# jinkakei/q-gcm

Hardware: AMD Instinct MI355X
Metric: ocean timesteps/sec (NAtl 5km 3-layer qgostep+ocinvq+ocqbdy) (higher is better)
Workload: dtype f64; 1 GPU; double_gyre_ocean_only NAtl 5km, 961x961x3 p-grid, dto=540s, Gaussian-eddy IC + double-gyre wind, oml off; parallelism=single GPU

## Files before the change

### q-gcm_amd/csrc/k_dst64.h

```cpp
#pragma once
#include "qgcm_dev.h"
#include "k_dst.h"
#include "k_misc.h"

#pragma clang fp contract(fast)

#ifndef D64_WAVES
#define D64_WAVES 2
#endif
#define D64_NT (64 * D64_WAVES)
#define D64_ROW 72

__device__ __forceinline__ void wave_lds_sync() {
  __builtin_amdgcn_fence(__ATOMIC_SEQ_CST, "wavefront");
  __builtin_amdgcn_wave_barrier();
}

__device__ __forceinline__ cplx cscale(cplx a, double s) { return {a.x * s, a.y * s}; }
__device__ __forceinline__ cplx cmpi(cplx a) { return {-a.y, a.x}; }

__device__ __forceinline__ void dft8(cplx *x) {
  const double r2 = 0.70710678118654752440;
  cplx e0 = cadd(x[0], x[4]), o0 = csub(x[0], x[4]);
  cplx e1 = cadd(x[1], x[5]), o1 = csub(x[1], x[5]);
// ... 73 lines not shown
  for (int ka = 0; ka < 3; ++ka)
#pragma unroll
    for (int kb = 0; kb < 5; ++kb) t[ka + 3 * kb] = a[5 * ka + kb];
#pragma unroll
  for (int k = 0; k < 15; ++k) a[k] = t[k];
}

template <int CTRL, int ROWMASK>
__device__ __forceinline__ double d64_dpp(double v) {
  int lo = __double2loint(v), hi = __double2hiint(v);
  lo = __builtin_amdgcn_update_dpp(0, lo, CTRL, ROWMASK, 0xf, true);
  hi = __builtin_amdgcn_update_dpp(0, hi, CTRL, ROWMASK, 0xf, true);
  return __hiloint2double(hi, lo);
}
__device__ __forceinline__ void d64_wave_scan2(double &a, double &b) {
  a += d64_dpp<0x111, 0xf>(a); b += d64_dpp<0x111, 0xf>(b);
  a += d64_dpp<0x112, 0xf>(a); b += d64_dpp<0x112, 0xf>(b);
  a += d64_dpp<0x114, 0xf>(a); b += d64_dpp<0x114, 0xf>(b);
  a += d64_dpp<0x118, 0xf>(a); b += d64_dpp<0x118, 0xf>(b);
  a += d64_dpp<0x142, 0xa>(a); b += d64_dpp<0x142, 0xa>(b);
  a += d64_dpp<0x143, 0xc>(a); b += d64_dpp<0x143, 0xc>(b);
}

template <int M>
__device__ __forceinline__ void dst64_front(const QgDstParams &P, const double *rowa, const double *rowb, bool has_b,
                                            cplx *F, cplx *W64, int lane) {
  constexpr int N = 64 * M, n = N - 1, NS2 = n / 2;

  cplx tw1[M];
  {
    double2 w = P.twid[lane];
    tw1[1 % M] = {w.x, w.y};
#pragma unroll
    for (int k1 = 2; k1 < M; ++k1) tw1[k1] = cmul(tw1[k1 / 2], tw1[k1 - k1 / 2]);
  }
  {
    double2 w = P.twid[M * lane];
    W64[lane] = {w.x, w.y};
  }

  constexpr int MH = M / 2;
  cplx a[M];
  {
    const double *rb = has_b ? rowb : rowa;
    const double bsc = has_b ? 1.0 : 0.0;
    double snv[MH + 1], xav[MH + 1], xac[MH + 1], xbv[MH + 1], xbc[MH + 1];
#pragma unroll
    for (int n1 = 0; n1 <= MH; ++n1) {
      const int j = 64 * n1 + lane;
      const int k = (j <= NS2 + 1) ? j : 0;
      const int i1 = k > 0 ? k - 1 : 0, i2 = k > 0 ? n - k : 0;
      snv[n1] = P.sintab[(k <= NS2) ? k : 0];
      xav[n1] = rowa[i1];
      xac[n1] = rowa[i2];
      xbv[n1] = rb[i1];
      xbc[n1] = rb[i2];
    }
    const int ml = (64 - lane) & 63;
#pragma unroll
    for (int n1 = 0; n1 <= MH; ++n1) {
      const int j = 64 * n1 + lane;
      const double va = xav[n1], ca = xac[n1], vb = bsc * xbv[n1], cb = bsc * xbc[n1];
      const double sn = snv[n1];
      const double t1a = va - ca, t2a = sn * (va + ca);
      const double t1b = vb - cb, t2b = sn * (vb + cb);
      cplx z = {t1a + t2a, t1b + t2b};
      if (j == NS2 + 1) z = {4.0 * va, 4.0 * vb};
      if (j == 0) z = {0.0, 0.0};
      a[n1] = z;
      if (j >= 1 && j <= NS2) {
        const int mn1 = (lane == 0) ? M - n1 : M - 1 - n1;
        F[mn1 * D64_ROW + ml + (ml >> 3)] = {t2a - t1a, t2b - t1b};
      }
    }
    wave_lds_sync();
#pragma unroll
    for (int n1 = MH; n1 < M; ++n1) {
      const int j = 64 * n1 + lane;
      const cplx zz = F[n1 * D64_ROW + lane + (lane >> 3)];
      if (j >= NS2 + 2) a[n1] = zz;
    }
    wave_lds_sync();
  }
  dftM<M>(a);
#pragma unroll
// ... 180 lines not shown
      const int t = lane + 64 * u;
      if (t < N / 2) {
        qg_store16_wt(rowa + 2 * t, oa[u].x, oa[u].y);
        if (has_b) qg_store16_wt(rowb + 2 * t, ob[u].x, ob[u].y);
      }
    }
  }
  QG_STAMP(0, 3);
  QG_STAMP_DRAIN();
  QG_STAMP(0, 4);
  if (ROWSUM) {
#pragma unroll
    for (int off = 32; off > 0; off >>= 1) {
      rsa += __shfl_down(rsa, off);
      rsb += __shfl_down(rsb, off);
    }
    if (lane == 0) {
      P.rowsum[(long)m * ny + (ja - 1)] = rsa;
      if (has_b) P.rowsum[(long)m * ny + ja] = rsb;
    }
  }
}

#pragma clang fp contract(off)

template <int M, int NL, bool BDY, bool HALO, bool CONSTR, bool AVG = false>
__global__ __launch_bounds__(64 * (NL + (CONSTR ? 1 : 0))) void k_dst64_unpack(const QgDstParams P, const QgUnpackParams U,
                                                                                      const QgBdyParams B, const QgConstrLite C) {
  constexpr int N = 64 * M, NP = N + N / 16;
  __shared__ __align__(16) cplx Fsh[NL][M * D64_ROW];
  __shared__ __align__(16) cplx W64sh[NL][64];
  __shared__ double hc_sh[NL];
  const int tid = threadIdx.x;
  const int lane = tid & 63;
  const int wv = __builtin_amdgcn_readfirstlane(tid >> 6);
  const int ldw = P.g.ldw;
  const int ja = P.g.jr0 + 2 * blockIdx.x;
  const bool has_b = (ja + 1 <= P.g.jr1);
  const long fs = U.g.fstride;
  const int nx = U.g.nx, nyg = U.g.nyg, joff = U.g.joff;
  constexpr int NX = N + 1;
  double hc[NL];
  const int jlo = U.g.jlo, jhi = U.g.jhi, ldxm = U.g.ldx;
  auto msg_p = [&](int gi, int gj, const double *pl) {
    if (HALO && U.msg_lo && gj - jlo < 3) {
#pragma unroll
      for (int k = 0; k < NL; ++k) U.msg_lo[((long)k * 3 + (gj - jlo)) * ldxm + (gi - 1)] = pl[k];
    }
    if (HALO && U.msg_hi && jhi - gj < 3) {
#pragma unroll
      for (int k = 0; k < NL; ++k) U.msg_hi[((long)k * 3 + (gj - (jhi - 2))) * ldxm + (gi - 1)] = pl[k];
    }
// ... 90 lines not shown
    constr_xin<NL>(C, lane, xin);
#pragma unroll
    for (int k = 0; k < NL - 1; ++k) dpn[k] = C.sc->dpioc[k];
    constr_box_solve<NL>(C, xin, dpn, x);
    if (lane == 0) {
#pragma unroll
      for (int m = 1; m < NL; ++m) hc_sh[m] = x[m - 1];
      if (blockIdx.x == 0) {
#pragma unroll
        for (int m = 0; m < NL; ++m) C.sc->xinhom[m] = xin[m];
#pragma unroll
        for (int k = 0; k < NL - 1; ++k) C.sc->hclco[k] = x[k];
      }
    }
    __syncthreads();
#pragma unroll
    for (int m = 1; m < NL; ++m) hc[m] = x[m - 1];
    if (lane < 2) wall_columns(lane, w);
    return;
  }
  constexpr int NT = 64 * NL, NPAIR = (NX - 3) / 2, NIT = (NPAIR + NT - 1) / NT;
  const double *rowa = P.wrk + P.g.wstride * wv + (long)(ja - 1) * ldw;
  QG_STAMP(2, 0);
  dst64_front<M>(P, rowa, rowa + ldw, has_b, Fsh[wv], W64sh[wv], lane);
  QG_STAMP(2, 1);
  asm volatile("" ::: "memory");
  double2 oc[2][NIT][NL - 1];
#pragma unroll
  for (int r = 0; r < 2; ++r)
#pragma unroll
    for (int it = 0; it < NIT; ++it) {
      const int q = tid + it * NT;
      const int gi = 3 + 2 * q;
      const bool ok = q < NPAIR && (r == 0 || has_b);
      const long o = (long)(ja + r - 1) * U.g.ldx + (gi - 1);
#pragma unroll
      for (int m = 1; m < NL; ++m) oc[r][it][m - 1] = ok ? *reinterpret_cast<const double2 *>(U.ochom + fs * (m - 1) + o) : double2{0.0, 0.0};
    }
  double2 pcv[AVG ? 2 : 1][AVG ? NIT : 1][AVG ? NL : 1];
  if (AVG) {
#pragma unroll
    for (int r = 0; r < 2; ++r)
#pragma unroll
      for (int it = 0; it < NIT; ++it) {
        const int q = tid + it * NT, qc = q < NPAIR ? q : 0;
        const long o = (long)(ja + ((r == 0 || has_b) ? r : 0) - 1) * U.g.ldx + (3 + 2 * qc - 1);
#pragma unroll
// ... 104 lines not shown
```

### q-gcm_amd/csrc/k_misc.h

```cpp
#pragma once
#include "qgcm_dev.h"

#define CS_NT 256

__device__ inline void qg_lu_solve(int n, const double *lu, const int *piv, double *b) {
  for (int k = 0; k < n; ++k)
    if (piv[k] != k) {
      double t = b[k];
      b[k] = b[piv[k]];
      b[piv[k]] = t;
    }
  for (int k = 0; k < n; ++k)
    for (int i = k + 1; i < n; ++i) b[i] -= lu[i + n * k] * b[k];
  for (int k = n - 1; k >= 0; --k) {
    b[k] /= lu[k + n * k];
    for (int i = 0; i < k; ++i) b[i] -= lu[i + n * k] * b[k];
  }
}

__device__ inline double qg_block_sum(double v, double *red, int tid) {
  red[tid] = v;
  __syncthreads();
  for (int off = CS_NT / 2; off > 0; off >>= 1) {
    if (tid < off) red[tid] += red[tid + off];
// ... 40 lines not shown
    double aitmp = sc->dpioc[k];
    sc->dpioc[k] = sc->dpiocp[k] - tdto * gpoc[k] * aient;
    sc->dpiocp[k] = aitmp;
  }
}

template <int NL, class PT>
__device__ __forceinline__ void constr_box_solve(const PT &P, const double *xin, const double *dpn, double *x) {
  constexpr int n1 = NL - 1;
  double rhs[n1], r[n1], w[n1];
#pragma unroll
  for (int k = 0; k < n1; ++k) {
    double rhsum = 0.0;
#pragma unroll
    for (int m = 0; m < NL; ++m) rhsum = rhsum + P.cs.cdiffo[m + NL * k] * xin[m];
    rhs[k] = dpn[k] - rhsum;
    x[k] = rhs[k];
  }
  auto lu_solve = [&](double *b) {
#pragma unroll
    for (int k = 0; k < n1; ++k) {
      const int pk = P.cs.ipiv[k];
#pragma unroll
      for (int i = 0; i < n1; ++i)
        if (i > k && i == pk) {
          double t = b[k];
          b[k] = b[i];
          b[i] = t;
        }
    }
#pragma unroll
    for (int k = 0; k < n1; ++k)
#pragma unroll
      for (int i = k + 1; i < n1; ++i) b[i] -= P.cs.cdhlu[i + n1 * k] * b[k];
#pragma unroll
    for (int k = n1 - 1; k >= 0; --k) {
      b[k] /= P.cs.cdhlu[k + n1 * k];
#pragma unroll
      for (int i = 0; i < k; ++i) b[i] -= P.cs.cdhlu[i + n1 * k] * b[k];
    }
  };
  lu_solve(x);
  const double eps = 1.1102230246251565e-16, safmin = 2.2250738585072014e-308;
  const double safe1 = (n1 + 1) * safmin, safe2 = safe1 / eps;
  double lstres = 3.0;
  for (int count = 1;; ++count) {
#pragma unroll
    for (int i = 0; i < n1; ++i) {
      double sv = rhs[i], t = fabs(rhs[i]);
#pragma unroll
      for (int j = 0; j < n1; ++j) {
        sv -= P.cs.cdhoc[i + n1 * j] * x[j];
// ... 261 lines not shown
```

### q-gcm_amd/csrc/k_thomas.h

```cpp
#pragma once
#include "qgcm_dev.h"
#include "k_cyclic.h"

#define TH_KW 16
#define TH_NC 64
#define TH_NT (TH_KW * TH_NC)
static_assert(TH_NC == 64, "the chunk scan maps the 64 chunks of a wavenumber to the lanes of one wave");

template <int CTRL>
__device__ __forceinline__ double th_dpp(double v) {
  int lo = __double2loint(v), hi = __double2hiint(v);
  lo = __builtin_amdgcn_update_dpp(lo, lo, CTRL, 0xf, 0xf, false);
  hi = __builtin_amdgcn_update_dpp(hi, hi, CTRL, 0xf, 0xf, false);
  return __hiloint2double(hi, lo);
}
template <int CTRL>
__device__ __forceinline__ void th_scan_step(double &Cs, double &Ds, bool take) {
  const double Cp = th_dpp<CTRL>(Cs), Dp = th_dpp<CTRL>(Ds);
  if (take) {
    Cs = Cs + Ds * Cp;
    Ds = Ds * Dp;
  }
}
__device__ __forceinline__ void affine_scan(double &Cs, double &Ds, int lane) {
  const int rl = lane & 15;
  th_scan_step<0x111>(Cs, Ds, rl >= 1);
  th_scan_step<0x112>(Cs, Ds, rl >= 2);
  th_scan_step<0x114>(Cs, Ds, rl >= 4);
  th_scan_step<0x118>(Cs, Ds, rl >= 8);
  th_scan_step<0x142>(Cs, Ds, (lane & 16) != 0);
  th_scan_step<0x143>(Cs, Ds, lane >= 32);
}

#define TH_MSG 3
#define TH_CST 4
template <int R, int PHASE, bool CYCA = false, int KW = TH_KW>
__global__ __launch_bounds__(KW * TH_NC, (KW == 8 && R <= 16) ? 4 : 1) void k_thomas(const QgThomasParams P) {
  static_assert(TH_KW % KW == 0, "a workgroup's wavenumbers lie inside one block of the pivot tables");
  static_assert(KW % 2 == 0, "the write-through stores pair the lanes of neighbouring wavenumbers");
  __shared__ double sC[TH_NC][KW + 1];
  __shared__ double sD[TH_NC][KW + 1];
  __shared__ double sIn[TH_NC][KW + 1];
  const int tid = threadIdx.x;
  if (CYCA && blockIdx.x == gridDim.x - 1) {
    if (P.cycq && blockIdx.y == 0 && tid < 64) {
      double a4[QG_MAXL], b4[QG_MAXL];
      switch (P.g.nl) {
        case 2: constr_cyc_partA<2>(*P.cycq, tid, a4, b4); break;
        case 3: constr_cyc_partA<3>(*P.cycq, tid, a4, b4); break;
        default: constr_cyc_partA<4>(*P.cycq, tid, a4, b4); break;
      }
    }
    return;
  }
  QG_STAMP(1, 0);
  int bxl = (int)blockIdx.x;
  if (KW == 8) {
    const int nfull = ((int)gridDim.x - (CYCA ? 1 : 0)) / 16 * 16;
    if (bxl < nfull) bxl = (bxl & ~15) + 2 * (bxl & 7) + ((bxl >> 3) & 1);
  }
  const int kk = tid % KW;
  const int c = tid / KW;
  const int lane = tid & 63, wv = tid >> 6;
  const int k = bxl * KW + kk;
  const int kq = bxl * KW + wv;
  const int m = blockIdx.y + P.layer0;
  const int nr = P.g.jr1 - P.g.jr0 + 1;
  const int ldw = P.g.ldw;
  const bool kok = k < P.g.nk;
  const double a = P.aoc;
  const int r0 = c * R;
  const long mk = TH_MSG * ((long)m * ldw + kq);
  const double ft = P.ftnorm;

  const double *wbase_c = P.wrk + P.g.wstride * m + (long)(P.g.jr0 - 1) * ldw + bxl * KW;
  double *wbase = const_cast<double *>(wbase_c);
  const unsigned off0 = (unsigned)(r0 * ldw + kk);
  constexpr bool PRED = (PHASE != 0);
  double w[R], b[R];
#pragma unroll
  for (int t = 0; t < R; ++t) {
    int r = r0 + t;
    const bool ok = kok && r < nr && PHASE != 4 && PHASE != 5;
    w[t] = ok ? wbase[off0 + (unsigned)(t * ldw)] : 0.0;
  }
  {
    const int tb = m * P.nblk + (bxl * KW) / TH_KW;
    const int rcb = P.rcb[tb];
    const double binf = kok ? P.binf[(long)m * ldw + k] : 0.0;
#pragma unroll
    for (int t = 0; t < R; ++t) b[t] = binf;
    if (r0 < rcb) {
      const double *tab = P.ptab + (long)P.poff[tb] * TH_KW + (bxl * KW) % TH_KW + kk;
#pragma unroll
      for (int t = 0; t < R; ++t) {
        const int r = r0 + t;
        const int rc = r < rcb ? r : rcb - 1;
        const double v = tab[rc * TH_KW];
        b[t] = (r < rcb && kok) ? v : binf;
      }
    }
    if (r0 + R > nr) {
#pragma unroll
      for (int t = 0; t < R; ++t)
        if (r0 + t >= nr) b[t] = 0.0;
    }
  }
// ... 49 lines not shown
  const int cr = 63 - lane;
  Cs = sC[cr][wv];
  Ds = sD[cr][wv];
  affine_scan(Cs, Ds, lane);
  const double Cb_tot = __shfl(Cs, 63);
  {
    double Cprev = th_dpp<0x138>(Cs), Dprev = th_dpp<0x138>(Ds);
    sIn[cr][wv] = (lane == 0) ? vin : Cprev + Dprev * vin;
  }
  __syncthreads();
  QG_STAMP(1, 5);
  double v = sIn[c][kk];
  double colsum = 0.0;
#pragma unroll
  for (int t = R - 1; t >= 0; --t) {
    if (!PRED || r0 + t < nr) {
      v = __builtin_fma(-b[t], v, w[t]);
      w[t] = v;
      colsum += v;
    }
  }
  QG_STAMP(1, 6);
  {
    if (R % 2 == 0) {
      const bool odd = (kk & 1) != 0;
      const bool pok = odd ? (k - 1 < P.g.nk) : kok;
      double *cbase = wbase + (odd ? off0 - 1 : off0);
#pragma unroll
      for (int t = 0; t < R; t += 2) {
        const double mine0 = ft * w[t], mine1 = ft * w[t + 1];
        const double give = odd ? mine0 : mine1;
        int lo = __double2loint(give), hi = __double2hiint(give);
        lo = __builtin_amdgcn_update_dpp(0, lo, 0xb1, 0xf, 0xf, true);
        hi = __builtin_amdgcn_update_dpp(0, hi, 0xb1, 0xf, 0xf, true);
        const double got = __hiloint2double(hi, lo);
        const int r = r0 + t + (odd ? 1 : 0);
        if (pok && r < nr) qg_store16_wt(cbase + (unsigned)((t + (odd ? 1 : 0)) * ldw), odd ? got : mine0, odd ? mine1 : got);
      }
    } else {
#pragma unroll
      for (int t = 0; t < R; ++t) {
        int r = r0 + t;
        if (kok && r < nr) wbase[off0 + (unsigned)(t * ldw)] = ft * w[t];
      }
    }
  }
  QG_STAMP(1, 7);
// ... 184 lines not shown
```

### q-gcm_amd/csrc/qgcm_hip.hip

```cpp
#include <hip/hip_runtime.h>
#include <cmath>
#include <cstdio>
#include <cstdlib>
#include <cstring>
#include <algorithm>
#include <map>
#include <vector>

#include "qgcm_dev.h"
#include "k_tend.h"
#include "k_dst.h"
#include "k_fft3.h"
#ifndef FFT3_NT
#define FFT3_NT 256
#endif
#ifdef FFT3_4800_OLD
#define QG_FFT3_PLANS(X) X(1, 15, 16, 20) X(2, 16, 16, 18) X(3, 16, 16, 16) X(4, 12, 15, 16)
#else
#define QG_FFT3_PLANS(X) X(1, 12, 20, 20) X(2, 16, 16, 18) X(3, 16, 16, 16) X(4, 12, 15, 16)
#endif
#include "k_dst64.h"
#include "k_thomas.h"
#include "k_misc.h"
#include "k_cyclic.h"
// ... 59 lines not shown
  return upto((long)s0 + n - 1) - upto((long)s0 - 1);
}
static int sched_dist(QgSched k, int s) { return k.every > 0 ? (k.phase - s % k.every + k.every) % k.every : kNeverDue; }
static int sched_set(QgSched &k, int every, int phase, const char *who) {
  if (every < 0) QG_FAIL("%s: every = %d (need >= 0; 0 removes the schedule)", who, every);
  if (every > 0 && (phase < 0 || phase >= every)) QG_FAIL("%s: phase = %d outside [0, %d)", who, phase, every);
  k.every = every;
  k.phase = every > 0 ? phase : 0;
  return 0;
}
enum { SCH_DUMP = 0, SCH_TAVATM, SCH_COV, SCH_COUNT };

struct qgcm_hip_ctx {
  qgcm_hip_params prm;
  QgGeom g;
  int device;
  hipStream_t stream;
  double *p[2], *q[2];
  int ip, iq;
  double *wekpo, *entoc, *ddynoc, *ochom, *yporel;
  double *rspl = nullptr;
  double c1_spl = 0.0;
  double *wrk, *rowsum;
  double *ybnd = nullptr;
  const double *slab_gath = nullptr;
  int slab_nranks = 1;
  const double *oml_gath = nullptr;
  double *bpart_out = nullptr;
  QgThomasTab tt, tt_tmp;
  struct {
    double *ptab = nullptr, *qtab = nullptr;
    int *meta = nullptr;
    size_t prows = 0, qrows = 0;
  } corr;
  double *slabDE;
  double *th_cgath = nullptr;
  int th_cgath_ranks = 0;
  double *ksum, *wcot;
  double *bpart;
  QgConstrParams *d_boxq = nullptr;
  QgCycConstrParams *d_cycq = nullptr;
  int thR;
  double *pch1, *pch2, *pbh;
  QgScalars *sc;
  double2 *twid;
  double *sintab;
  int fftN, nfac, fac[QG_MAXFAC];
  QgConstr cs;
  bool grid_set, homog_set;
  bool geom_set = false;
  bool whole;
  bool dst_single = false;
  int fft3 = 0;
  size_t fft3_lds = 0;
  bool force_generic_dst;
  bool no_fused_unpack;
  int cu_first = 0, cu_count = 0;
  bool no_fused_avg;
  bool avg_now = false;
  bool no_fused_constr;
  bool tend_wide;
  std::vector<double> bd2oc;
  hipError_t timer_err = hipSuccess;
  int timer_err_at = 0;
  bool profiling;
  hipEvent_t ev0, ev1;
  std::vector<hipEvent_t> evpool;
  std::vector<int> evkid;
  double kms[KN_COUNT];
  int klaunch[KN_COUNT];
  struct GraphEntry { hipGraphExec_t exec; unsigned long used; };
  std::map<long long, GraphEntry> graphs;
  unsigned long graph_call = 0;
  int avg_period = 25;
  struct {
    bool on = false;
    qgcm_hip_oml_params prm;
    int ldt = 0, is = 0, ism = 1, nblkA = 0, nblkB = 0;
    double *sst[3] = {nullptr, nullptr, nullptr};
    double *fnet = nullptr, *wekto = nullptr, *xfo = nullptr, *taux = nullptr, *tauy = nullptr;
    double *partA = nullptr, *partB = nullptr, *diag = nullptr;
// ... 195 lines not shown
  if (dalloc(&c->slabDE, (size_t)4 * g.ldw * g.nl)) return 1;
  if (g.cyc && dalloc(&c->ybnd, 2 * QG_MAXL)) return 1;
  if (dalloc(&c->ksum, (size_t)g.ldw * g.nl)) return 1;
  if (dalloc(&c->wcot, (size_t)g.ldw)) return 1;
  if (dalloc(&c->bpart, (size_t)5 * BSUM_NB * 2 * g.nl)) return 1;
  if (dalloc(&c->rowsum, (size_t)g.ny * g.nl)) return 1;
  if (dalloc(&c->pch1, (size_t)g.ny * g.nl) || dalloc(&c->pch2, (size_t)g.ny * g.nl) || dalloc(&c->pbh, g.ny)) return 1;
  HIPCHECK(hipMalloc((void **)&c->sc, sizeof(QgScalars)));
  HIPCHECK(hipMemset(c->sc, 0, sizeof(QgScalars)));
  c->twid = nullptr;
  c->sintab = nullptr;
  c->grid_set = c->homog_set = false;
  {
    const char *e = getenv("QGCM_HIP_GENERIC_DST");
    c->force_generic_dst = e && e[0] == '1';
    const char *f = getenv("QGCM_HIP_NO_FUSED_UNPACK");
    c->no_fused_unpack = f && f[0] == '1';
    const char *fc = getenv("QGCM_HIP_NO_FUSED_CONSTR");
    c->no_fused_constr = fc && fc[0] == '1';
    const char *tw = getenv("QGCM_HIP_TEND_WIDE");
    c->tend_wide = tw && tw[0] == '1';
    const char *fa = getenv("QGCM_HIP_NO_FUSED_AVG");
    c->no_fused_avg = fa && fa[0] == '1';
  }
  c->profiling = false;
  HIPCHECK(hipEventCreate(&c->ev0));
  HIPCHECK(hipEventCreate(&c->ev1));
  memset(&c->cs, 0, sizeof(c->cs));
  HIPCHECK(hipDeviceSynchronize());
  *h = c;
  return 0;
}

extern "C" int qgcm_hip_destroy(qgcm_hip_handle c) {
  if (!c) return 0;
  hipStreamSynchronize(c->stream);
  for (auto &kv : c->graphs) hipGraphExecDestroy(kv.second.exec);
  for (auto &kv : c->slab_graphs) hipGraphExecDestroy(kv.second);
  if (c->sc_comm) {
    QgSlabComm *m = c->sc_comm;
    if (m->comm) m->api->CommDestroy(m->comm);
    if (m->ev_fork) hipEventDestroy(m->ev_fork);
    if (m->ev_halo) hipEventDestroy(m->ev_halo);
    if (m->cstream) hipStreamDestroy(m->cstream);
    double *cb[] = {m->th_send, m->th_gath, m->h_send, m->h_gath, m->oml_send, m->oml_gath};
    for (double *p : cb)
// ... 49 lines not shown
    if (p) hipFree(p);
  if (c->twid) hipFree(c->twid);
  hipFree(c->sc);
  if (c->d_cycq) hipFree(c->d_cycq);
  if (c->d_boxq) hipFree(c->d_boxq);
  if (c->corr.ptab) hipFree(c->corr.ptab);
  if (c->corr.qtab) hipFree(c->corr.qtab);
  if (c->corr.meta) hipFree(c->corr.meta);
  for (QgThomasTab *t : {&c->tt, &c->tt_tmp}) {
    if (t->binf) hipFree(t->binf);
    if (t->ptab) hipFree(t->ptab);
    if (t->rcb) hipFree(t->rcb);
    if (t->poff) hipFree(t->poff);
  }
  hipEventDestroy(c->ev0);
  hipEventDestroy(c->ev1);
  for (hipEvent_t e : c->evpool) hipEventDestroy(e);
  hipStreamDestroy(c->stream);
  delete c;
  return 0;
}

#define QG_TH_ROWS(X) X(1) X(2) X(4) X(8) X(10) X(12) X(16) X(20) X(24) X(32)
static int thomas_rows_per_chunk(int nrows) {
  const int need = (nrows + TH_NC - 1) / TH_NC;
#define QG_TH_FITS(RV) if (need <= RV) return RV;
  QG_TH_ROWS(QG_TH_FITS)
#undef QG_TH_FITS
  return -1;
}

static inline size_t slab_msg_len(const QgGeom &g) {
  return (size_t)TH_MSG * g.nl * g.ldw + (g.cyc ? (size_t)5 * BSUM_NB * 2 * g.nl : 0);
}
static inline size_t slab_msg_len_oml(const qgcm_hip_ctx *c) { return slab_msg_len(c->g) + (c->oml.on ? 3 : 0); }
static inline size_t halo_msg_len(const qgcm_hip_ctx *c) {
  return (size_t)4 * c->g.nl * c->g.ldx + (c->oml.on ? (size_t)3 * c->oml.ldt : 0);
}

struct ThomasTabHost {
  std::vector<double> binf, ptab;
  std::vector<int> rcb, poff;
};
static void build_pivots(const QgGeom &g, double aoc, const double *boc , ThomasTabHost &T) {
  const int nr = g.jr1 - g.jr0 + 1;
  const int rg0 = g.jr0 + g.joff - 2;
// ... 32 lines not shown
static int upload_pivots(qgcm_hip_ctx *c, QgThomasTab &D, const ThomasTabHost &T) {
  auto fit = [&](void **p, size_t &cap, size_t n, size_t el) -> int {
    if (n <= cap && *p) return 0;
    if (*p) HIPCHECK(hipFree(*p));
    *p = nullptr;
    HIPCHECK(hipMalloc(p, n * el));
    cap = n;
    return 0;
  };
  HIPCHECK(hipStreamSynchronize(c->stream));
  if (fit((void **)&D.binf, D.binf_n, T.binf.size(), sizeof(double))) return 1;
  if (fit((void **)&D.ptab, D.ptab_n, T.ptab.size(), sizeof(double))) return 1;
  if (fit((void **)&D.rcb, D.rcb_n, T.rcb.size(), sizeof(int))) return 1;
  if (fit((void **)&D.poff, D.poff_n, T.poff.size(), sizeof(int))) return 1;
  HIPCHECK(hipMemcpy(D.binf, T.binf.data(), T.binf.size() * sizeof(double), hipMemcpyHostToDevice));
  HIPCHECK(hipMemcpy(D.ptab, T.ptab.data(), T.ptab.size() * sizeof(double), hipMemcpyHostToDevice));
  HIPCHECK(hipMemcpy(D.rcb, T.rcb.data(), T.rcb.size() * sizeof(int), hipMemcpyHostToDevice));
  HIPCHECK(hipMemcpy(D.poff, T.poff.data(), T.poff.size() * sizeof(int), hipMemcpyHostToDevice));
  return 0;
}

static int launch_thomas(qgcm_hip_ctx *c, double *wrk, const QgThomasTab &tab, int nlayers, int phase,
                         const double *gath, double *send, int rank, int nranks, int layer0, hipStream_t st,
                         bool cyc_part_a = false);

static void fill_thomas_params(qgcm_hip_ctx *c, QgThomasParams &P, double *wrk, const QgThomasTab &tab, int nlayers, int layer0) {
  const QgGeom &g = c->g;
  memset(&P, 0, sizeof(P));
  P.g = g;
  P.gath_stride = (long)slab_msg_len_oml(c);
  P.slabDE = c->slabDE;
  P.ksum = c->ksum;
  P.wrk = wrk;
  P.binf = tab.binf; P.ptab = tab.ptab; P.rcb = tab.rcb; P.poff = tab.poff;
  P.nblk = (g.nk + TH_KW - 1) / TH_KW;
  P.aoc = c->prm.aoc;
  P.ftnorm = g.cyc ? 1.0 / g.nxt : 0.5 / g.nxt;
  P.nlayers = nlayers;
  P.layer0 = layer0;
  P.nranks = 1;
}

static int build_slab_responses(qgcm_hip_ctx *c) {
  const QgGeom &g = c->g;
  const int nblk = (g.nk + TH_KW - 1) / TH_KW, nm = nblk * g.nl;
  const bool nb_lo = g.joff + g.jlo > 1, nb_hi = g.joff + g.jhi < g.nyg;
  if (!c->corr.meta) HIPCHECK(hipMalloc((void **)&c->corr.meta, sizeof(int) * 4 * nm));
// ... 458 lines not shown
  F.cyc = c->g.cyc; F.on = on ? 1 : 0;
  F.sc = c->sc;
  F.ocnorm = 1.0 / ((double)c->g.nxt * (double)(c->g.nyg - 1));
  F.dxo = c->prm.dxo; F.dyo = c->prm.dyo;
}

enum { TEND_ALL = 0, TEND_INNER = 1, TEND_OUTER = 2 };
static bool tend_can_split(const qgcm_hip_ctx *c) {
  const TendTiling T = c->g.cyc ? tend_tiling<true>(c->g) : tend_tiling<false>(c->g);
  return T.gy >= 3;
}

enum { ROWS_GENERIC = 0, ROWS_DST64, ROWS_RFFT64, ROWS_FFT3 };
enum { INV_PLAIN = 0, INV_DST64_UNPACK, INV_RFFT64_UNPACK, INV_FFT3_UNPACK };
enum { CONSTR_OWN = 0, CONSTR_INV_WAVE, CONSTR_BOX_WG, CONSTR_AB };
struct QgStepPlan {
  int rows;
  int m64;
  int inv;
  int constr;
  bool upd_dpi;
  bool wtq;
  bool avg_ok;
};

static QgStepPlan step_plan(const qgcm_hip_ctx *c, bool in_step = false, bool slab = false) {
  const QgGeom &g = c->g;
  QgStepPlan pl;
  const int N = c->fftN;
  pl.m64 = c->force_generic_dst ? 0 : (N == 64 * 3 ? 3 : N == 64 * 15 ? 15 : (g.cyc && N == 64 * 6) ? 6 : 0);
  pl.rows = (c->fft3 && !c->force_generic_dst) ? ROWS_FFT3 : pl.m64 ? (g.cyc ? ROWS_RFFT64 : ROWS_DST64) : ROWS_GENERIC;
  pl.inv = INV_PLAIN;
  if (!c->no_fused_unpack) {
    if (pl.rows == ROWS_DST64 && g.nl <= 4) pl.inv = INV_DST64_UNPACK;
    if (pl.rows == ROWS_RFFT64 && g.nl <= 4 && c->whole && !slab) pl.inv = INV_RFFT64_UNPACK;
    if (pl.rows == ROWS_FFT3 && g.cyc && !g.atm && g.nl == 3 && g.ldx % 2 == 0) pl.inv = INV_FFT3_UNPACK;
  }
  pl.constr = CONSTR_OWN;
  if (!c->no_fused_constr) {
    if (g.cyc) {
      if (in_step && !slab && g.nl <= 4 && (pl.inv == INV_RFFT64_UNPACK || pl.rows != ROWS_RFFT64)) pl.constr = CONSTR_AB;
    } else if (pl.inv == INV_DST64_UNPACK) {
      if (in_step && !(slab && c->oml.on)) pl.constr = CONSTR_INV_WAVE;
    } else if (pl.rows != ROWS_DST64 && g.nl <= 3) {
      pl.constr = CONSTR_BOX_WG;
    }
  }
  if (pl.inv == INV_FFT3_UNPACK && !slab && pl.constr != CONSTR_AB) pl.inv = INV_PLAIN;
  pl.upd_dpi = pl.constr == CONSTR_INV_WAVE;
  pl.wtq = (double)g.fstride * 8.0 * (7 * g.nl - 1) < 200.0e6 && !c->tend_wide;
  pl.avg_ok = in_step && !slab && !c->no_fused_avg && !c->poavg.on &&
              ((pl.constr == CONSTR_INV_WAVE && pl.wtq) || pl.inv == INV_FFT3_UNPACK);
  return pl;
}

static int launch_tend(qgcm_hip_ctx *c, bool upd_dpi = false, bool oml_final = false, int part = TEND_ALL) {
  const QgGeom &g = c->g;
  const qgcm_hip_params &pr = c->prm;
  QgTendParams P;
  memset(&P, 0, sizeof(P));
  P.g = g;
  P.pom = c->p[c->ip ^ 1];
  P.po = c->p[c->ip];
  P.qo = c->q[c->iq];
  P.qnew = c->q[c->iq ^ 1];
  P.wekpo = c->wekpo; P.entoc = c->entoc; P.ddynoc = c->ddynoc; P.yporel = c->yporel;
  P.wrk = c->wrk; P.sc = c->sc; P.bsum = nullptr;
  P.adfaco = 1.0 / (12.0 * pr.dxo * pr.dyo * pr.fnot);
  P.dxom2 = 1.0 / (pr.dxo * pr.dxo);
  P.bcfaco = pr.bccooc * P.dxom2 / (0.5 * pr.bccooc + 1.0);
  P.tdto = pr.tdto;
  P.bdrfac = 0.5 * (pr.fnot >= 0.0 ? 1.0 : -1.0) * pr.delek / pr.hoc[g.nl - 1];
// ... 107 lines not shown
    const int M64 = pl.m64;
#define QG_RF(MV)                                                                           \
  if (inverse) hipLaunchKernelGGL((k_rfft64<MV, true>), grid64, dim3(D64_NT), 0, st, P);    \
  else hipLaunchKernelGGL((k_rfft64<MV, false>), grid64, dim3(D64_NT), 0, st, P)
    if (M64 == 3) { QG_RF(3); }
    else if (M64 == 6) { QG_RF(6); }
    else if (M64 == 15) { QG_RF(15); }
    else if (inverse) hipLaunchKernelGGL((k_rfft_cyc<true>), grid, dim3(RFFT_NT), c->dst_lds, st, P);
    else hipLaunchKernelGGL((k_rfft_cyc<false>), grid, dim3(RFFT_NT), c->dst_lds, st, P);
#undef QG_RF
    HIPCHECK(hipGetLastError());
    return 0;
  }
  if (pl.m64 == 15) {
    hipLaunchKernelGGL((k_dst64<15, false>), grid64, dim3(D64_NT), 0, st, P);
  } else if (pl.m64 == 3) {
    hipLaunchKernelGGL((k_dst64<3, false>), grid64, dim3(D64_NT), 0, st, P);
  } else if (c->fftN >= DST_BIG_N) hipLaunchKernelGGL((k_dst_box<false, DST_NT_BIG>), grid, dim3(DST_NT_BIG), c->dst_lds, st, P);
  else hipLaunchKernelGGL((k_dst_box<false>), grid, dim3(DST_NT), c->dst_lds, st, P);
  HIPCHECK(hipGetLastError());
  return 0;
}

static int launch_thomas(qgcm_hip_ctx *c, double *wrk, const QgThomasTab &tab, int nlayers, int phase,
                         const double *gath, double *send, int rank, int nranks, int layer0, hipStream_t st,
                         bool cyc_part_a) {
  if (!st) st = c->stream;
  const QgGeom &g = c->g;
  if (!tab.binf) QG_FAIL("k_thomas: the pivot tables have not been built (qgcm_hip_set_grid)");
  QgThomasParams P;
  fill_thomas_params(c, P, wrk, tab, nlayers, layer0);
  P.gath = gath; P.send = send; P.rank = rank; P.nranks = nranks;
  if (phase == 2) {
    if (g.cyc) P.ybnd = c->ybnd;
    c->slab_gath = gath;
    c->slab_nranks = nranks;
    P.cgath = (nranks == 1) ? c->slabDE : c->th_cgath;
    if (nranks > 1 && (!c->th_cgath || c->th_cgath_ranks != nranks))
      QG_FAIL("qgcm_hip_thomas_phase: the set-up constants of the %d slabs have not been exchanged (qgcm_hip_set_thomas_consts)", nranks);
    if (&tab != &c->tt || !c->corr.meta) QG_FAIL("k_thomas_corr: the response tables belong to the modal solves of qgcm_hip_set_grid");
    const int nm = P.nblk * g.nl;
    QgThomasCorr T;
    T.ptab = c->corr.ptab; T.qtab = c->corr.qtab;
    T.np = c->corr.meta; T.nq = c->corr.meta + nm; T.poff = c->corr.meta + 2 * nm; T.qoff = c->corr.meta + 3 * nm;
    KTimer t(c, KN_THOMAS, st);
    const size_t lds = sizeof(double) * THC_LDS * nranks;
    if (lds > 32 * 1024)
      HIPCHECK(hipFuncSetAttribute((const void *)k_thomas_corr, hipFuncAttributeMaxDynamicSharedMemorySize, (int)lds));
    const int nrows = g.jr1 - g.jr0 + 1, per = THC_UNR * (THC_NT / 8);
    hipLaunchKernelGGL(k_thomas_corr, dim3(P.nblk, nlayers, (nrows + per - 1) / per), dim3(THC_NT), lds, st, P, T);
    HIPCHECK(hipGetLastError());
    return 0;
  }
  if (phase == 0) {
    c->slab_gath = nullptr;
    if (g.cyc && nlayers == g.nl) P.ybnd = c->ybnd;
  }
  const bool cyca = (phase == 0 && g.cyc);
  if (cyc_part_a && (phase != 0 || !c->d_cycq || g.nl > 4)) QG_FAIL("k_thomas: part A of the constraint algebra needs the homogeneous solutions and nlo <= 4");
  if (cyca) P.cycq = cyc_part_a ? c->d_cycq : nullptr;
  KTimer t(c, KN_THOMAS, st);
#define QG_TH(RV, KWV)                                                                                                  \
  {                                                                                                                      \
    dim3 gridk((g.nk + KWV - 1) / KWV + (cyca ? 1 : 0), nlayers);                                                        \
    switch (phase) {                                                                                                     \
      case 0:                                                                                                            \
        if (cyca) hipLaunchKernelGGL((k_thomas<RV, 0, true, KWV>), gridk, dim3(KWV * TH_NC), 0, st, P);                  \
        else hipLaunchKernelGGL((k_thomas<RV, 0, false, KWV>), gridk, dim3(KWV * TH_NC), 0, st, P);                      \
        break;                                                                                                           \
      case 1: hipLaunchKernelGGL((k_thomas<RV, 1, false, KWV>), gridk, dim3(KWV * TH_NC), 0, st, P); break;              \
      case 4: hipLaunchKernelGGL((k_thomas<RV, 4, false, KWV>), gridk, dim3(KWV * TH_NC), 0, st, P); break;              \
      default: hipLaunchKernelGGL((k_thomas<RV, 5, false, KWV>), gridk, dim3(KWV * TH_NC), 0, st, P); break;             \
    }                                                                                                                    \
  }
  switch (c->thR) {
#define QG_TH_CASE(RV) case RV: QG_TH(RV, 8); break;
    QG_TH_ROWS(QG_TH_CASE)
#undef QG_TH_CASE
    default: QG_FAIL("k_thomas: too many rows for the single-segment kernel");
  }
#undef QG_TH
  HIPCHECK(hipGetLastError());
  return 0;
}
// ... 121 lines not shown
  fill_dst_params(c, D, c->wrk, g.nl, 0);
  QgUnpackParams P;
  if (fill_unpack_params(c, P, msg_lo, msg_hi, "k_rfft3_unpack", own_constr)) return 1;
  QgBdyParams B;
  fill_bdy_params(c, B);
  const int npairs = (g.jr1 - g.jr0 + 2) / 2;
  dim3 grid(8 * ((npairs + 7) / 8) * g.nl);
  KTimer t(c, KN_DSTI);
  QgCycConstrParams Q;
  fill_cyc_constr_params(c, Q);
#define QG_FFT3U_LAUNCH(ID, R1, R2, R3)                                                                                   \
  if (c->fft3 == ID) {                                                                                                    \
    typedef Fft3Plan<R1, R2, R3> PL;                                                                                      \
    if (c->avg_now) hipLaunchKernelGGL((k_rfft3_unpack<PL, 3, FFT3_NT, true>), grid, dim3(FFT3_NT), c->fft3_lds, c->stream, D, P, B, Q, 1); \
    else hipLaunchKernelGGL((k_rfft3_unpack<PL, 3, FFT3_NT>), grid, dim3(FFT3_NT), c->fft3_lds, c->stream, D, P, B, Q, own_constr ? 1 : 0); \
  }
  QG_FFT3_PLANS(QG_FFT3U_LAUNCH)
#undef QG_FFT3U_LAUNCH
  HIPCHECK(hipGetLastError());
  return 0;
}

static int launch_dst_unpack(qgcm_hip_ctx *c, bool fuse_bdy, double *msg_lo = nullptr, double *msg_hi = nullptr,
                             bool constr = false) {
  const QgGeom &g = c->g;
  QgDstParams D;
  fill_dst_params(c, D, c->wrk, g.nl, 0);
  QgUnpackParams P;
  if (fill_unpack_params(c, P, msg_lo, msg_hi, "k_dst64_unpack", fuse_bdy && constr)) return 1;
  QgBdyParams B;
  fill_bdy_params(c, B);
  QgConstrLite C;
  fill_constr_lite(c, C);
  const int nrows = g.jr1 - g.jr0 + 1;
  dim3 grid((nrows + 1) / 2);
  KTimer t(c, KN_DSTI);
#define QG_DU(MV, NLV)                                                                                                  \
  if (c->avg_now) hipLaunchKernelGGL((k_dst64_unpack<MV, NLV, true, false, true, true>), grid, dim3(64 * (NLV + 1)), 0, c->stream, D, P, B, C); \
  else if ((msg_lo || msg_hi) && constr) hipLaunchKernelGGL((k_dst64_unpack<MV, NLV, true, true, true>), grid, dim3(64 * (NLV + 1)), 0, c->stream, D, P, B, C); \
  else if (msg_lo || msg_hi) hipLaunchKernelGGL((k_dst64_unpack<MV, NLV, true, true, false>), grid, dim3(64 * NLV), 0, c->stream, D, P, B, C); \
  else if (fuse_bdy && constr) hipLaunchKernelGGL((k_dst64_unpack<MV, NLV, true, false, true>), grid, dim3(64 * (NLV + 1)), 0, c->stream, D, P, B, C); \
  else if (fuse_bdy) hipLaunchKernelGGL((k_dst64_unpack<MV, NLV, true, false, false>), grid, dim3(64 * NLV), 0, c->stream, D, P, B, C);  \
  else hipLaunchKernelGGL((k_dst64_unpack<MV, NLV, false, false, false>), grid, dim3(64 * NLV), 0, c->stream, D, P, B, C)
#define QG_DU_NL(MV)                 \
  switch (g.nl) {                    \
    case 2: QG_DU(MV, 2); break;     \
    case 3: QG_DU(MV, 3); break;     \
    default: QG_DU(MV, 4); break;    \
  }
  if (step_plan(c).m64 == 15) {
    QG_DU_NL(15)
  } else {
    QG_DU_NL(3)
  }
#undef QG_DU_NL
#undef QG_DU
  HIPCHECK(hipGetLastError());
  return 0;
}

static int launch_ocqbdy(qgcm_hip_ctx *c) {
// ... 17 lines not shown
  HIPCHECK(hipGetLastError());
  return 0;
}

static int check_ready(qgcm_hip_ctx *c, const char *who) {
  if (!c) QG_FAIL("%s: null handle", who);
  if (!c->grid_set) QG_FAIL("%s: qgcm_hip_set_grid has not been called", who);
  return 0;
}

extern "C" int qgcm_hip_qgostep(qgcm_hip_handle c) {
  if (check_ready(c, "qgcm_hip_qgostep")) return 1;
  if (launch_tend(c)) return 1;
  c->iq ^= 1;
  return 0;
}

static int ocinvq_impl(qgcm_hip_ctx *c, bool in_step = false) {
  if (check_ready(c, "qgcm_hip_ocinvq")) return 1;
  if (!c->whole) QG_FAIL("qgcm_hip_ocinvq: this handle is a y-slab; drive it with the slab building blocks");
  if (!c->homog_set) QG_FAIL("qgcm_hip_ocinvq: homogeneous solutions not set");
  const QgStepPlan pl = step_plan(c, in_step);
  const bool fuse_bdy = in_step;
  if (launch_dst(c, c->wrk, c->g.nl, false)) return 1;
  if (launch_thomas(c, c->wrk, c->tt, c->g.nl, 0, nullptr, nullptr, 0, 1, 0, nullptr, pl.constr == CONSTR_AB)) return 1;
  if (pl.constr == CONSTR_OWN && launch_constr(c)) return 1;
  switch (pl.inv) {
    case INV_DST64_UNPACK:
      if (launch_dst_unpack(c, fuse_bdy, nullptr, nullptr, pl.constr == CONSTR_INV_WAVE)) return 1;
      break;
    case INV_RFFT64_UNPACK:
      if (launch_rfft_unpack(c, fuse_bdy, pl.constr == CONSTR_AB)) return 1;
      break;
    case INV_FFT3_UNPACK:
      if (launch_fft3_unpack(c, true)) return 1;
      break;
    default:
      if (launch_dst(c, c->wrk, c->g.nl, true, 0, nullptr, pl.constr == CONSTR_AB, pl.constr == CONSTR_BOX_WG)) return 1;
      if (launch_unpack(c, fuse_bdy)) return 1;
  }
  c->ip ^= 1;
  return 0;
}

extern "C" int qgcm_hip_ocinvq(qgcm_hip_handle c) { return ocinvq_impl(c); }

extern "C" int qgcm_hip_ocqbdy(qgcm_hip_handle c) {
  if (check_ready(c, "qgcm_hip_ocqbdy")) return 1;
  return launch_ocqbdy(c);
}

extern "C" int qgcm_hip_ocqbdy_host(qgcm_hip_handle c, double *q, const double *p) {
// ... 1718 lines not shown
```

Before: 15350 steps/s.

## Store spectral work array row-pair interleaved across forward DST, Thomas and inverse DST

Adds a pair-interleaved layout for the spectral work array. A new forward DST kernel writes two rows per wavenumber as a single 16-byte store, and the Thomas solve and the fused inverse-DST unpack then read and write those pairs with double2 accesses. The aim is fewer, wider, more coalesced memory transactions across the three stages of the elliptic inversion. It also replaces the pivot-swap loop in the constraint solve with branchless selects. The cost is extra template instantiations, and the path is limited to whole-domain box grids with eligible sizes, with an environment-variable opt-out.

```diff
diff --git a/q-gcm_amd/csrc/k_dst64.h b/q-gcm_amd/csrc/k_dst64.h
--- a/q-gcm_amd/csrc/k_dst64.h
+++ b/q-gcm_amd/csrc/k_dst64.h
@@ -119,7 +119,7 @@
   a += d64_dpp<0x143, 0xc>(a); b += d64_dpp<0x143, 0xc>(b);
 }
 
-template <int M>
+template <int M, bool BLK = false>
 __device__ __forceinline__ void dst64_front(const QgDstParams &P, const double *rowa, const double *rowb, bool has_b,
                                             cplx *F, cplx *W64, int lane) {
   constexpr int N = 64 * M, n = N - 1, NS2 = n / 2;
@@ -148,16 +148,25 @@
       const int k = (j <= NS2 + 1) ? j : 0;
       const int i1 = k > 0 ? k - 1 : 0, i2 = k > 0 ? n - k : 0;
       snv[n1] = P.sintab[(k <= NS2) ? k : 0];
-      xav[n1] = rowa[i1];
-      xac[n1] = rowa[i2];
-      xbv[n1] = rb[i1];
-      xbc[n1] = rb[i2];
+      if (BLK) {
+        const double2 v1 = *reinterpret_cast<const double2 *>(rowa + 2 * i1);
+        const double2 v2 = *reinterpret_cast<const double2 *>(rowa + 2 * i2);
+        xav[n1] = v1.x;
+        xac[n1] = v2.x;
+        xbv[n1] = has_b ? v1.y : 0.0;
+        xbc[n1] = has_b ? v2.y : 0.0;
+      } else {
+        xav[n1] = rowa[i1];
+        xac[n1] = rowa[i2];
+        xbv[n1] = rb[i1];
+        xbc[n1] = rb[i2];
+      }
     }
     const int ml = (64 - lane) & 63;
 #pragma unroll
     for (int n1 = 0; n1 <= MH; ++n1) {
       const int j = 64 * n1 + lane;
-      const double va = xav[n1], ca = xac[n1], vb = bsc * xbv[n1], cb = bsc * xbc[n1];
+      const double va = xav[n1], ca = xac[n1], vb = BLK ? xbv[n1] : bsc * xbv[n1], cb = BLK ? xbc[n1] : bsc * xbc[n1];
       const double sn = snv[n1];
       const double t1a = va - ca, t2a = sn * (va + ca);
       const double t1b = vb - cb, t2b = sn * (vb + cb);
@@ -384,12 +393,44 @@
   }
 }
 
+template <int M>
+__global__ __launch_bounds__(D64_NT) void k_dst64_blk(const QgDstParams P) {
+  constexpr int N = 64 * M;
+  __shared__ __align__(16) cplx Fsh[D64_WAVES][M * D64_ROW];
+  __shared__ __align__(16) cplx W64sh[D64_WAVES][64];
+  const int lane = threadIdx.x & 63;
+  const int wv = __builtin_amdgcn_readfirstlane(threadIdx.x >> 6);
+  const int ldw = P.g.ldw;
+  const int m = blockIdx.y + P.layer0;
+  const int pair = blockIdx.x * D64_WAVES + wv;
+  const int ja = P.g.jr0 + 2 * pair;
+  if (ja > P.g.jr1) return;
+  const bool has_b = (ja + 1 <= P.g.jr1);
+  double *dst = P.wrk + P.g.wstride * m + (long)(ja - 1) * ldw;
+  const double *rowa = dst;
+  double rsa, rsb;
+  dst64_front<M>(P, rowa, rowa + ldw, has_b, Fsh[wv], W64sh[wv], lane);
+  dst64_back<M>(Fsh[wv], W64sh[wv], lane, rsa, rsb);
+  const double *raw = reinterpret_cast<const double *>(Fsh[wv]);
+  constexpr int NP = N + N / 16;
+  double oa[M], ob[M];
+#pragma unroll
+  for (int u = 0; u < M; ++u) {
+    const int k = lane + 64 * u, i = k + (k >> 4);
+    oa[u] = raw[i];
+    ob[u] = raw[NP + i];
+  }
+#pragma unroll
+  for (int u = 0; u < M; ++u) qg_store16_wt(dst + 2 * (lane + 64 * u), oa[u], has_b ? ob[u] : 0.0);
+}
+
 #pragma clang fp contract(off)
 
-template <int M, int NL, bool BDY, bool HALO, bool CONSTR, bool AVG = false>
+template <int M, int NL, bool BDY, bool HALO, bool CONSTR, bool AVG = false, bool BLK = false>
 __global__ __launch_bounds__(64 * (NL + (CONSTR ? 1 : 0))) void k_dst64_unpack(const QgDstParams P, const QgUnpackParams U,
                                                                                       const QgBdyParams B, const QgConstrLite C) {
   constexpr int N = 64 * M, NP = N + N / 16;
+  static_assert(!BLK || !HALO, "the pair-interleaved spectral form belongs to whole-domain handles");
   __shared__ __align__(16) cplx Fsh[NL][M * D64_ROW];
   __shared__ __align__(16) cplx W64sh[NL][64];
   __shared__ double hc_sh[NL];
@@ -526,7 +567,7 @@
   constexpr int NT = 64 * NL, NPAIR = (NX - 3) / 2, NIT = (NPAIR + NT - 1) / NT;
   const double *rowa = P.wrk + P.g.wstride * wv + (long)(ja - 1) * ldw;
   QG_STAMP(2, 0);
-  dst64_front<M>(P, rowa, rowa + ldw, has_b, Fsh[wv], W64sh[wv], lane);
+  dst64_front<M, BLK>(P, rowa, rowa + ldw, has_b, Fsh[wv], W64sh[wv], lane);
   QG_STAMP(2, 1);
   asm volatile("" ::: "memory");
   double2 oc[2][NIT][NL - 1];
diff --git a/q-gcm_amd/csrc/k_misc.h b/q-gcm_amd/csrc/k_misc.h
--- a/q-gcm_amd/csrc/k_misc.h
+++ b/q-gcm_amd/csrc/k_misc.h
@@ -86,12 +86,12 @@
     for (int k = 0; k < n1; ++k) {
       const int pk = P.cs.ipiv[k];
 #pragma unroll
-      for (int i = 0; i < n1; ++i)
-        if (i > k && i == pk) {
-          double t = b[k];
-          b[k] = b[i];
-          b[i] = t;
-        }
+      for (int i = k + 1; i < n1; ++i) {
+        const bool sw = (i == pk);
+        const double bk = b[k], bi = b[i];
+        b[k] = sw ? bi : bk;
+        b[i] = sw ? bk : bi;
+      }
     }
 #pragma unroll
     for (int k = 0; k < n1; ++k)
diff --git a/q-gcm_amd/csrc/k_thomas.h b/q-gcm_amd/csrc/k_thomas.h
--- a/q-gcm_amd/csrc/k_thomas.h
+++ b/q-gcm_amd/csrc/k_thomas.h
@@ -34,9 +34,10 @@
 
 #define TH_MSG 3
 #define TH_CST 4
-template <int R, int PHASE, bool CYCA = false, int KW = TH_KW>
+template <int R, int PHASE, bool CYCA = false, int KW = TH_KW, bool BLK = false>
 __global__ __launch_bounds__(KW * TH_NC, (KW == 8 && R <= 16) ? 4 : 1) void k_thomas(const QgThomasParams P) {
   static_assert(TH_KW % KW == 0, "a workgroup's wavenumbers lie inside one block of the pivot tables");
+  static_assert(!BLK || (PHASE == 0 && !CYCA), "only the whole-column box solve has the pair-interleaved form");
   static_assert(KW % 2 == 0, "the write-through stores pair the lanes of neighbouring wavenumbers");
   __shared__ double sC[TH_NC][KW + 1];
   __shared__ double sD[TH_NC][KW + 1];
@@ -73,16 +74,28 @@
   const long mk = TH_MSG * ((long)m * ldw + kq);
   const double ft = P.ftnorm;
 
-  const double *wbase_c = P.wrk + P.g.wstride * m + (long)(P.g.jr0 - 1) * ldw + bxl * KW;
+  const int BP = 2 * ldw;
+  const double *wbase_c = BLK ? P.wrk + P.g.wstride * m + (long)(P.g.jr0 - 1) * ldw + bxl * (2 * KW)
+                              : P.wrk + P.g.wstride * m + (long)(P.g.jr0 - 1) * ldw + bxl * KW;
   double *wbase = const_cast<double *>(wbase_c);
-  const unsigned off0 = (unsigned)(r0 * ldw + kk);
+  const unsigned off0 = BLK ? (unsigned)((r0 >> 1) * BP + 2 * kk + (r0 & 1)) : (unsigned)(r0 * ldw + kk);
   constexpr bool PRED = (PHASE != 0);
   double w[R], b[R];
-#pragma unroll
-  for (int t = 0; t < R; ++t) {
-    int r = r0 + t;
-    const bool ok = kok && r < nr && PHASE != 4 && PHASE != 5;
-    w[t] = ok ? wbase[off0 + (unsigned)(t * ldw)] : 0.0;
+  if (BLK && R % 2 == 0) {
+#pragma unroll
+    for (int t = 0; t < R; t += 2) {
+      const int r = r0 + t;
+      const double2 v = (kok && r < nr) ? *reinterpret_cast<const double2 *>(wbase_c + off0 + (unsigned)(t / 2 * BP)) : double2{0.0, 0.0};
+      w[t] = v.x;
+      w[t + 1] = (r + 1 < nr) ? v.y : 0.0;
+    }
+  } else {
+#pragma unroll
+    for (int t = 0; t < R; ++t) {
+      int r = r0 + t;
+      const bool ok = kok && r < nr && PHASE != 4 && PHASE != 5;
+      w[t] = ok ? wbase[off0 + (BLK ? (unsigned)(((r >> 1) - (r0 >> 1)) * BP + (r & 1) - (r0 & 1)) : (unsigned)(t * ldw))] : 0.0;
+    }
   }
   {
     const int tb = m * P.nblk + (bxl * KW) / TH_KW;
@@ -178,7 +191,19 @@
   }
   QG_STAMP(1, 6);
   {
-    if (R % 2 == 0) {
+    if (BLK && R % 2 == 0) {
+#pragma unroll
+      for (int t = 0; t < R; t += 2) {
+        const int r = r0 + t;
+        if (kok && r < nr) qg_store16_wt(wbase + off0 + (unsigned)(t / 2 * BP), ft * w[t], (r + 1 < nr) ? ft * w[t + 1] : 0.0);
+      }
+    } else if (BLK) {
+#pragma unroll
+      for (int t = 0; t < R; ++t) {
+        const int r = r0 + t;
+        if (kok && r < nr) wbase[off0 + (unsigned)(((r >> 1) - (r0 >> 1)) * BP + (r & 1) - (r0 & 1))] = ft * w[t];
+      }
+    } else if (R % 2 == 0) {
       const bool odd = (kk & 1) != 0;
       const bool pok = odd ? (k - 1 < P.g.nk) : kok;
       double *cbase = wbase + (odd ? off0 - 1 : off0);
diff --git a/q-gcm_amd/csrc/qgcm_hip.hip b/q-gcm_amd/csrc/qgcm_hip.hip
--- a/q-gcm_amd/csrc/qgcm_hip.hip
+++ b/q-gcm_amd/csrc/qgcm_hip.hip
@@ -105,6 +105,7 @@
   double *rspl = nullptr;
   double c1_spl = 0.0;
   double *wrk, *rowsum;
+  bool blk_ok = false;
   double *ybnd = nullptr;
   const double *slab_gath = nullptr;
   int slab_nranks = 1;
@@ -140,6 +141,7 @@
   bool no_fused_unpack;
   int cu_first = 0, cu_count = 0;
   bool no_fused_avg;
+  bool no_blocked_spectral = false;
   bool avg_now = false;
   bool no_fused_constr;
   bool tend_wide;
@@ -381,6 +383,13 @@
     c->tend_wide = tw && tw[0] == '1';
     const char *fa = getenv("QGCM_HIP_NO_FUSED_AVG");
     c->no_fused_avg = fa && fa[0] == '1';
+    const char *nb = getenv("QGCM_HIP_NO_BLOCKED_SPECTRAL");
+    c->no_blocked_spectral = nb && nb[0] == '1';
+  }
+  {
+    const int nrows = g.jr1 - g.jr0 + 1;
+    c->blk_ok = !c->no_blocked_spectral && !g.cyc && c->whole && (g.nxt == 64 * 3 || g.nxt == 64 * 15) && g.nl >= 2 && g.nl <= 4 &&
+                nrows <= 16 * TH_NC && g.jr0 - 1 + 2 * ((nrows + 1) / 2) <= g.ny && 2 * g.nxt <= 2 * g.ldw;
   }
   c->profiling = false;
   HIPCHECK(hipEventCreate(&c->ev0));
@@ -476,6 +485,7 @@
 }
 
 #define QG_TH_ROWS(X) X(1) X(2) X(4) X(8) X(10) X(12) X(16) X(20) X(24) X(32)
+#define QG_TH_ROWS_BLK(X) X(1) X(2) X(4) X(8) X(10) X(12) X(16)
 static int thomas_rows_per_chunk(int nrows) {
   const int need = (nrows + TH_NC - 1) / TH_NC;
 #define QG_TH_FITS(RV) if (need <= RV) return RV;
@@ -554,7 +564,7 @@
 
 static int launch_thomas(qgcm_hip_ctx *c, double *wrk, const QgThomasTab &tab, int nlayers, int phase,
                          const double *gath, double *send, int rank, int nranks, int layer0, hipStream_t st,
-                         bool cyc_part_a = false);
+                         bool cyc_part_a = false, bool blk = false);
 
 static void fill_thomas_params(qgcm_hip_ctx *c, QgThomasParams &P, double *wrk, const QgThomasTab &tab, int nlayers, int layer0) {
   const QgGeom &g = c->g;
@@ -1059,6 +1069,7 @@
   bool upd_dpi;
   bool wtq;
   bool avg_ok;
+  bool blk;
 };
 
 static QgStepPlan step_plan(const qgcm_hip_ctx *c, bool in_step = false, bool slab = false) {
@@ -1085,6 +1096,7 @@
   }
   if (pl.inv == INV_FFT3_UNPACK && !slab && pl.constr != CONSTR_AB) pl.inv = INV_PLAIN;
   pl.upd_dpi = pl.constr == CONSTR_INV_WAVE;
+  pl.blk = pl.inv == INV_DST64_UNPACK && !slab && c->whole && c->blk_ok;
   pl.wtq = (double)g.fstride * 8.0 * (7 * g.nl - 1) < 200.0e6 && !c->tend_wide;
   pl.avg_ok = in_step && !slab && !c->no_fused_avg && !c->poavg.on &&
               ((pl.constr == CONSTR_INV_WAVE && pl.wtq) || pl.inv == INV_FFT3_UNPACK);
@@ -1238,9 +1250,24 @@
   return 0;
 }
 
+static int launch_dst_blk(qgcm_hip_ctx *c) {
+  const QgGeom &g = c->g;
+  const QgStepPlan pl = step_plan(c);
+  if (!pl.blk) QG_FAIL("k_dst64_blk: not a whole-domain box handle of the wave-per-row-pair rows");
+  QgDstParams P;
+  fill_dst_params(c, P, c->wrk, g.nl, 0);
+  const int npairs = (g.jr1 - g.jr0 + 2) / 2;
+  dim3 grid64((npairs + D64_WAVES - 1) / D64_WAVES, g.nl);
+  KTimer t(c, KN_DSTF);
+  if (pl.m64 == 15) hipLaunchKernelGGL((k_dst64_blk<15>), grid64, dim3(D64_NT), 0, c->stream, P);
+  else hipLaunchKernelGGL((k_dst64_blk<3>), grid64, dim3(D64_NT), 0, c->stream, P);
+  HIPCHECK(hipGetLastError());
+  return 0;
+}
+
 static int launch_thomas(qgcm_hip_ctx *c, double *wrk, const QgThomasTab &tab, int nlayers, int phase,
                          const double *gath, double *send, int rank, int nranks, int layer0, hipStream_t st,
-                         bool cyc_part_a) {
+                         bool cyc_part_a, bool blk) {
   if (!st) st = c->stream;
   const QgGeom &g = c->g;
   if (!tab.binf) QG_FAIL("k_thomas: the pivot tables have not been built (qgcm_hip_set_grid)");
@@ -1276,6 +1303,19 @@
   if (cyc_part_a && (phase != 0 || !c->d_cycq || g.nl > 4)) QG_FAIL("k_thomas: part A of the constraint algebra needs the homogeneous solutions and nlo <= 4");
   if (cyca) P.cycq = cyc_part_a ? c->d_cycq : nullptr;
   KTimer t(c, KN_THOMAS, st);
+  if (blk) {
+    if (phase != 0 || cyca || !c->blk_ok || wrk != c->wrk || nlayers != g.nl || layer0 != 0 || &tab != &c->tt)
+      QG_FAIL("k_thomas: the pair-interleaved form belongs to the whole-column modal solves of a box ocean");
+    const dim3 gridk((g.nk + 7) / 8, nlayers);
+    switch (c->thR) {
+#define QG_TH_BLK(RV) case RV: hipLaunchKernelGGL((k_thomas<RV, 0, false, 8, true>), gridk, dim3(8 * TH_NC), 0, st, P); break;
+      QG_TH_ROWS_BLK(QG_TH_BLK)
+#undef QG_TH_BLK
+      default: QG_FAIL("k_thomas: %d rows per thread have no blocked instantiation", c->thR);
+    }
+    HIPCHECK(hipGetLastError());
+    return 0;
+  }
 #define QG_TH(RV, KWV)                                                                                                  \
   {                                                                                                                      \
     dim3 gridk((g.nk + KWV - 1) / KWV + (cyca ? 1 : 0), nlayers);                                                        \
@@ -1443,10 +1483,11 @@
 }
 
 static int launch_dst_unpack(qgcm_hip_ctx *c, bool fuse_bdy, double *msg_lo = nullptr, double *msg_hi = nullptr,
-                             bool constr = false) {
+                             bool constr = false, bool blk = false) {
   const QgGeom &g = c->g;
   QgDstParams D;
   fill_dst_params(c, D, c->wrk, g.nl, 0);
+  if (blk && (msg_lo || msg_hi || !c->blk_ok)) QG_FAIL("k_dst64_unpack: the pair-interleaved form belongs to whole-domain handles");
   QgUnpackParams P;
   if (fill_unpack_params(c, P, msg_lo, msg_hi, "k_dst64_unpack", fuse_bdy && constr)) return 1;
   QgBdyParams B;
@@ -1457,7 +1498,11 @@
   dim3 grid((nrows + 1) / 2);
   KTimer t(c, KN_DSTI);
 #define QG_DU(MV, NLV)                                                                                                  \
-  if (c->avg_now) hipLaunchKernelGGL((k_dst64_unpack<MV, NLV, true, false, true, true>), grid, dim3(64 * (NLV + 1)), 0, c->stream, D, P, B, C); \
+  if (blk && c->avg_now) hipLaunchKernelGGL((k_dst64_unpack<MV, NLV, true, false, true, true, true>), grid, dim3(64 * (NLV + 1)), 0, c->stream, D, P, B, C); \
+  else if (blk && fuse_bdy && constr) hipLaunchKernelGGL((k_dst64_unpack<MV, NLV, true, false, true, false, true>), grid, dim3(64 * (NLV + 1)), 0, c->stream, D, P, B, C); \
+  else if (blk && fuse_bdy) hipLaunchKernelGGL((k_dst64_unpack<MV, NLV, true, false, false, false, true>), grid, dim3(64 * NLV), 0, c->stream, D, P, B, C); \
+  else if (blk) hipLaunchKernelGGL((k_dst64_unpack<MV, NLV, false, false, false, false, true>), grid, dim3(64 * NLV), 0, c->stream, D, P, B, C); \
+  else if (c->avg_now) hipLaunchKernelGGL((k_dst64_unpack<MV, NLV, true, false, true, true>), grid, dim3(64 * (NLV + 1)), 0, c->stream, D, P, B, C); \
   else if ((msg_lo || msg_hi) && constr) hipLaunchKernelGGL((k_dst64_unpack<MV, NLV, true, true, true>), grid, dim3(64 * (NLV + 1)), 0, c->stream, D, P, B, C); \
   else if (msg_lo || msg_hi) hipLaunchKernelGGL((k_dst64_unpack<MV, NLV, true, true, false>), grid, dim3(64 * NLV), 0, c->stream, D, P, B, C); \
   else if (fuse_bdy && constr) hipLaunchKernelGGL((k_dst64_unpack<MV, NLV, true, false, true>), grid, dim3(64 * (NLV + 1)), 0, c->stream, D, P, B, C); \
@@ -1521,12 +1566,12 @@
   if (!c->homog_set) QG_FAIL("qgcm_hip_ocinvq: homogeneous solutions not set");
   const QgStepPlan pl = step_plan(c, in_step);
   const bool fuse_bdy = in_step;
-  if (launch_dst(c, c->wrk, c->g.nl, false)) return 1;
-  if (launch_thomas(c, c->wrk, c->tt, c->g.nl, 0, nullptr, nullptr, 0, 1, 0, nullptr, pl.constr == CONSTR_AB)) return 1;
+  if (pl.blk ? launch_dst_blk(c) : launch_dst(c, c->wrk, c->g.nl, false)) return 1;
+  if (launch_thomas(c, c->wrk, c->tt, c->g.nl, 0, nullptr, nullptr, 0, 1, 0, nullptr, pl.constr == CONSTR_AB, pl.blk)) return 1;
   if (pl.constr == CONSTR_OWN && launch_constr(c)) return 1;
   switch (pl.inv) {
     case INV_DST64_UNPACK:
-      if (launch_dst_unpack(c, fuse_bdy, nullptr, nullptr, pl.constr == CONSTR_INV_WAVE)) return 1;
+      if (launch_dst_unpack(c, fuse_bdy, nullptr, nullptr, pl.constr == CONSTR_INV_WAVE, pl.blk)) return 1;
       break;
     case INV_RFFT64_UNPACK:
       if (launch_rfft_unpack(c, fuse_bdy, pl.constr == CONSTR_AB)) return 1;
```

After: 15180 steps/s. 0.989x the previous value.
